# earth-insights/ZoomEarth

Hardware: AMD Instinct MI355X
Metric: questions/sec end-to-end, ZoomEarth-3B on 5000px tiles (higher is better)
Workload: dtype bf16

## Files before the change

### zoomearth_amd/csrc/ze_elementwise.hip

```cpp
#include <hip/hip_fp16.h>

#include "ze_kernels.h"
#include "ze_prng.h"

__device__ __forceinline__ int map_row(int r, int mode, int offset) {
    return mode == 0 ? offset + r : (r >> 4) * 32 + (r & 15) + offset;
}

__global__ void __launch_bounds__(256) k_pack_rows(const void* __restrict__ src, int dtype, int row0, int nrows,
                                                   int cols, bf16_t* __restrict__ dst, int ld, int mode, int offset) {
    const size_t i = (size_t)blockIdx.x * 256 + threadIdx.x;
    if (i >= (size_t)nrows * cols) return;
    const int r = (int)(i / cols), c = (int)(i % cols);
    bf16_t v;
    if (dtype == ZE_BF16) {
        v = ((const bf16_t*)src)[i];
    } else if (dtype == ZE_F16) {
        v = f32_to_bf16(__half2float(((const __half*)src)[i]));
    } else {
        v = f32_to_bf16(((const float*)src)[i]);
    }
    dst[(size_t)map_row(row0 + r, mode, offset) * ld + c] = v;
}

// ... 401 lines not shown
}
void ze_launch_mrope_kv(bf16_t* qkv, int T, int heads, int kv_heads, int D, const bf16_t* cosT, const bf16_t* sinT,
                        const int* pos3, const int* axis_of, bf16_t* kcache, bf16_t* vcache, int max_ctx, int past,
                        const int* row_aux, size_t cache_seq_stride, hipStream_t s, int q_skip) {
    const size_t total = (size_t)T * (heads + 2 * kv_heads) * (D / 2);
    if (total == 0) return;
    if (D % 16 == 0 && mrope_vec_ok) {
        const size_t tv = (size_t)T * (q_skip ? 2 * kv_heads : heads + 2 * kv_heads) * (D / 2) / 8;
        k_mrope_kv_vec<<<(unsigned)((tv + 255) / 256), 256, 0, s>>>(qkv, T, heads, kv_heads, D, cosT, sinT, pos3, axis_of, kcache,
                                                                  vcache, max_ctx, past, row_aux, cache_seq_stride, q_skip);
        return;
    }
    k_mrope_kv<<<(unsigned)((total + 255) / 256), 256, 0, s>>>(qkv, T, heads, kv_heads, D, cosT, sinT, pos3,
                                                               axis_of, kcache, vcache, max_ctx, past, row_aux,
                                                               cache_seq_stride);
}

__global__ void __launch_bounds__(256) k_embed_rows(const int* __restrict__ src, const bf16_t* __restrict__ embed,
                                                    const bf16_t* __restrict__ image_embeds,
                                                    bf16_t* __restrict__ out, int T, int hidden) {
    const int nv = hidden >> 3;
    const size_t i = (size_t)blockIdx.x * 256 + threadIdx.x;
    if (i >= (size_t)T * nv) return;
    const int t = (int)(i / nv), v = (int)(i % nv);
    const int sidx = src[t];
    const bf16_t* row = sidx >= 0 ? embed + (size_t)sidx * hidden : image_embeds + (size_t)(-1 - sidx) * hidden;
    *reinterpret_cast<uint4*>(out + (size_t)t * hidden + v * 8) = *reinterpret_cast<const uint4*>(row + v * 8);
}
void ze_launch_embed_rows(const int* src, const bf16_t* embed, const bf16_t* image_embeds, bf16_t* out, int T,
                          int hidden, hipStream_t s) {
    const size_t n = (size_t)T * (hidden / 8);
    if (n == 0) return;
    k_embed_rows<<<(unsigned)((n + 255) / 256), 256, 0, s>>>(src, embed, image_embeds, out, T, hidden);
}

__global__ void __launch_bounds__(256) k_scatter_rows(const bf16_t* __restrict__ src, int lds_,
                                                      const int* __restrict__ dst_idx, bf16_t* __restrict__ dst,
                                                      int ldd, int rows, int cols) {
    const int nv = cols >> 3;
    const size_t i = (size_t)blockIdx.x * 256 + threadIdx.x;
    if (i >= (size_t)rows * nv) return;
    const int r = (int)(i / nv), v = (int)(i % nv);
    const int d = dst_idx ? dst_idx[r] : r;
    *reinterpret_cast<uint4*>(dst + (size_t)d * ldd + v * 8) =
        *reinterpret_cast<const uint4*>(src + (size_t)r * lds_ + v * 8);
}
void ze_launch_scatter_rows(const bf16_t* src, int lds_, const int* dst_idx, bf16_t* dst, int ldd, int rows,
                            int cols, hipStream_t s) {
    const size_t n = (size_t)rows * (cols / 8);
    if (n == 0) return;
    k_scatter_rows<<<(unsigned)((n + 255) / 256), 256, 0, s>>>(src, lds_, dst_idx, dst, ldd, rows, cols);
}

__global__ void __launch_bounds__(256) k_embed_tokens_batch(const ze_seq_dev* __restrict__ st,
                                                            const int* __restrict__ seq_ids, int n,
                                                            const bf16_t* __restrict__ embed, bf16_t* __restrict__ out,
                                                            int hidden) {
    const int nv = hidden >> 3;
    const size_t i = (size_t)blockIdx.x * 256 + threadIdx.x;
    if (i >= (size_t)n * nv) return;
    const int b = (int)(i / nv), v = (int)(i % nv);
    const int tok = st[seq_ids[b]].token;
    *reinterpret_cast<uint4*>(out + (size_t)b * hidden + v * 8) =
        *reinterpret_cast<const uint4*>(embed + (size_t)tok * hidden + v * 8);
}
struct ze_int_pack {
    int v[128];
};
__global__ void k_set_ints(int* __restrict__ dst, ze_int_pack p, int n) {
    const int i = threadIdx.x;
    if (i < n) dst[i] = p.v[i];
}
void ze_launch_set_ints(int* dst, const int* host_vals, int n, hipStream_t s) {
    for (int o = 0; o < n; o += 128) {
        ze_int_pack p;
        const int m = n - o < 128 ? n - o : 128;
        for (int i = 0; i < 128; ++i) p.v[i] = i < m ? host_vals[o + i] : 0;
        hipLaunchKernelGGL(k_set_ints, dim3(1), dim3(128), 0, s, dst + o, p, m);
    }
}

__global__ void k_scatter_ints(int* __restrict__ dst, ze_int_pack p, int n) {
    const int i = threadIdx.x;
    if (i < n) dst[p.v[i]] = p.v[64 + i];
}
void ze_launch_scatter_ints(int* dst, const int* host_idx, const int* host_vals, int n, hipStream_t s) {
    for (int o = 0; o < n; o += 64) {
        ze_int_pack p;
        const int m = n - o < 64 ? n - o : 64;
        for (int i = 0; i < 64; ++i) {
            p.v[i] = i < m ? host_idx[o + i] : 0;
            p.v[64 + i] = i < m ? host_vals[o + i] : 0;
        }
        hipLaunchKernelGGL(k_scatter_ints, dim3(1), dim3(64), 0, s, dst, p, m);
    }
}

void ze_launch_embed_tokens_batch(const ze_seq_dev* st, const int* seq_ids, int n, const bf16_t* embed, bf16_t* out,
                                  int hidden, hipStream_t s) {
    const size_t tot = (size_t)n * (hidden / 8);
    if (tot == 0) return;
    k_embed_tokens_batch<<<(unsigned)((tot + 255) / 256), 256, 0, s>>>(st, seq_ids, n, embed, out, hidden);
}

__global__ void __launch_bounds__(256) k_rope_kv_batch(bf16_t* __restrict__ qkv, int n, int heads, int kv_heads, int D,
                                                       const bf16_t* __restrict__ cosT, const bf16_t* __restrict__ sinT,
// ... 109 lines not shown
```

### zoomearth_amd/csrc/ze_engine.h

```cpp
#pragma once
#include <algorithm>
#include <map>
#include <tuple>
#include <set>
#include <string>
#include <vector>

#include "ze_host.h"
#include "ze_kernels.h"

struct ze_linear {
    bf16_t* w = nullptr;
    bf16_t* bias = nullptr;
    int n = 0, k = 0, ld = 0;
    uint8_t* w8 = nullptr;
    float* scale8 = nullptr;
    int ld8 = 0;
    bf16_t* wf = nullptr;
    bf16_t* wp = nullptr;
    bf16_t* bias_p = nullptr;
    uint8_t* wf8 = nullptr;
};
struct ze_vit_block {
    bf16_t *norm1 = nullptr, *norm2 = nullptr;
// ... 201 lines not shown
    struct ev_pair { int phase; hipEvent_t a, b; };
    std::vector<ev_pair> ev_used;
    std::vector<ev_pair> ev_free;
    float phase_ms[5] = {0, 0, 0, 0, 0};

    bf16_t* kc(int layer, int seq) const {
        return kcache + (((size_t)layer * cfg.max_seqs + seq) * cfg.kv_heads) * (size_t)cfg.max_ctx * head_dim;
    }
    bf16_t* vc(int layer, int seq) const {
        return vcache + (((size_t)layer * cfg.max_seqs + seq) * cfg.kv_heads) * (size_t)cfg.max_ctx * head_dim;
    }
};

#define ZE_TRY(x)               \
    do {                        \
        int _r = (x);           \
        if (_r != 0) return _r; \
    } while (0)
#define ZE_KCHECK() ZE_HIP(hipGetLastError())

extern unsigned ze_tune_epoch;
void ze_weights_changed(ze_engine* e);
int ze_engine_build_layout(ze_engine* e);
int ze_timer_begin(ze_engine* e, int phase, hipStream_t s);
void ze_timer_end(ze_engine* e, int handle, hipStream_t s);

template <typename T>
static int dev_alloc(ze_engine* e, T** p, size_t count, bool zero = true) {
    ZE_HIP(hipMalloc((void**)p, std::max<size_t>(count, 1) * sizeof(T)));
    if (zero) ZE_HIP(hipMemset(*p, 0, std::max<size_t>(count, 1) * sizeof(T)));
    return 0;
}
static inline int check_seq(ze_engine* e, int seq) {
    if (!e) return ze_fail(e, ZE_ERR_INVALID, "null engine");
    if (seq < 0 || seq >= e->cfg.max_seqs) return ze_fail(e, ZE_ERR_NOTFOUND, "sequence id out of range");
    return ZE_OK;
}

#pragma GCC visibility push(hidden)
int ze_requests_create(ze_engine* e);
void ze_requests_free(ze_engine* e);
void ze_requests_clear(ze_engine* e, int seq, hipStream_t s);
const float* ze_requests_rows(ze_engine* e, const float* logits, const int* seq_ids, int slot0, int n, hipStream_t s);
void ze_requests_logprobs(ze_engine* e, const float* logits, const int* seq_ids, int slot0, int n, hipStream_t s);
void ze_requests_after_token(ze_engine* e, const float* logits, const int* seq_ids, int slot0, int n, hipStream_t s);
int ze_check_filter(ze_engine* e, int top_k, float top_p, float min_p);
void ze_attach_filters(ze_engine* e, ze_sample_opts& so, bool batch);
float ze_penalty_of(const ze_engine* e, const ze_gen_params* p, int seq);
ze_sample_opts ze_sample_opts_of(ze_engine* e, const ze_gen_params* p, int slot, bool batch = false);
ze_step_key ze_step_key_of(const ze_engine* e, int n, int seq, float penalty, int ignore_eos, const ze_sample_opts& so);

enum { ZE_PROJ_QKV = 0, ZE_PROJ_O = 1, ZE_PROJ_GATE_UP = 2, ZE_PROJ_DOWN = 3 };
enum { ZE_NORM_IN = 0, ZE_NORM_POST = 1, ZE_NORM_FINAL = 2 };
void prefill_projection(ze_engine* e, const ze_text_layer& L, int which, int rows, bool norm, bf16_t* out, int ldo, hipStream_t s);
ze_gemv_args gemv_args_of(const ze_engine* e, const ze_linear& lin, int N, int K, const bf16_t* x);
ze_linear lm_head_linear(const ze_engine* e, bool decode);
void batch_norm(ze_engine* e, int li, int n, int which, hipStream_t s);
bool batch_qkv(ze_engine* e, int li, int n, hipStream_t s);
void batch_attention(ze_engine* e, int li, int n, hipStream_t s);
bool batch_o(ze_engine* e, int li, int n, hipStream_t s);
bool batch_gate_up(ze_engine* e, int li, int n, hipStream_t s);
bool batch_down(ze_engine* e, int li, int n, hipStream_t s);
bool batch_lm_head(ze_engine* e, int li, int n, hipStream_t s);
int ensure_fragments(ze_engine* e, hipStream_t s);
void sync_prefix(ze_engine* e, const int32_t* seqs, int n, hipStream_t s);
void upload_mates(ze_engine* e, const int32_t* seqs, int n, hipStream_t s);
void set_live_parts(ze_engine* e, const int32_t* seqs, int n, int steps);
#pragma GCC visibility pop
```

### zoomearth_amd/csrc/ze_engine.hip

```cpp
#include <math.h>
#include <string.h>

#include "ze_engine.h"
#include "ze_prng.h"

thread_local std::string ze_global_error;
extern int ze_mrope_vec_ok;
unsigned ze_tune_epoch = 0;
extern int ze_live_engines;
static int ze_bound_device = -1;

void ze_weights_changed(ze_engine* e) {
    e->frag_ready = false;
    if (e->fp8_ready) {
        e->fp8_ready = false;
        e->fp8_act = false;
        for (auto& L : e->tl)
            for (ze_linear* l : {&L.qkv, &L.o, &L.gate_up, &L.down}) {
                l->w8 = nullptr;
                l->scale8 = nullptr;
                l->wf8 = nullptr;
            }
        e->lm_head8.w8 = nullptr;
        e->lm_head8.scale8 = nullptr;
// ... 245 lines not shown
    e->graphs.assign(c.max_seqs, nullptr);
    e->graph_key.assign(c.max_seqs, ze_step_key{});
    chk(ze_requests_create(e));

    const size_t side = (size_t)std::max(c.max_tile_side, 1024);
    e->fe_tmp_bytes = side * 4096 * 3;
    e->fe_img_bytes = (size_t)4096 * 4096 * 3;
    chk(dev_alloc(e, &e->fe_tmp, e->fe_tmp_bytes, false));
    chk(dev_alloc(e, &e->fe_img, e->fe_img_bytes, false));
    e->fe_coef_ints = (size_t)4096 * 96 * 2 + 4096 * 4;
    chk(dev_alloc(e, &e->fe_coef, e->fe_coef_ints, false));
    if (r == 0 && hipHostMalloc((void**)&e->fe_coef_host, e->fe_coef_ints * sizeof(int)) != hipSuccess)
        r = ze_fail(e, ZE_ERR_HIP, "hipHostMalloc failed");

    const size_t np = c.max_patches;
    const int vh = c.vit_hidden, mu = c.spatial_merge_size * c.spatial_merge_size;
    const int pk = c.in_channels * c.temporal_patch_size * c.patch_size * c.patch_size;
    chk(dev_alloc(e, &e->vx, np * pk));
    chk(dev_alloc(e, &e->vh, np * vh));
    chk(dev_alloc(e, &e->vy, np * vh));
    chk(dev_alloc(e, &e->vqkv, np * 3 * vh));
    chk(dev_alloc(e, &e->vo, np * vh));
    chk(dev_alloc(e, &e->va, np * e->vit_ipad));
    chk(dev_alloc(e, &e->vz, np / mu * (size_t)vh * mu + 8));
    chk(dev_alloc(e, &e->vz2, np / mu * (size_t)c.vit_out_hidden + 8));
    chk(dev_alloc(e, &e->vcos, np * (e->vit_head_dim / 2)));
    chk(dev_alloc(e, &e->vsin, np * (e->vit_head_dim / 2)));
    chk(dev_alloc(e, &e->vperm, np));
    chk(dev_alloc(e, &e->vinv, np));
    chk(dev_alloc(e, &e->vtiles_win, np));
    chk(dev_alloc(e, &e->vtiles_full, np));
    e->v_host_ints_cap = np * 2 + np * 4 * 2 + 64;
    e->v_host_f32_cap = np * e->vit_head_dim;
    if (r == 0 && (hipHostMalloc((void**)&e->v_host_ints, e->v_host_ints_cap * sizeof(int)) != hipSuccess ||
                   hipHostMalloc((void**)&e->v_host_f32, e->v_host_f32_cap * sizeof(float)) != hipSuccess))
        r = ze_fail(e, ZE_ERR_HIP, "hipHostMalloc failed");

    const size_t tm = std::max(c.max_ctx, c.max_prefill_rows);
    e->prefill_rows = (int)tm;
    const int nqkv = (c.heads + 2 * c.kv_heads) * e->head_dim;
    chk(dev_alloc(e, &e->th, tm * c.hidden));
    chk(dev_alloc(e, &e->ty, tm * c.hidden));
    chk(dev_alloc(e, &e->ty8p, tm * c.hidden, false));
    chk(dev_alloc(e, &e->ty8p_scale, tm, false));
    chk(dev_alloc(e, &e->damax, 2 * 2048));
    if (r == 0 && e->damax) ze_launch_amax_init(e->damax, nullptr);
    chk(dev_alloc(e, &e->ty8, (size_t)64 * c.hidden));
    chk(dev_alloc(e, &e->ty8_scale, 64));
    chk(dev_alloc(e, &e->tqkv, tm * nqkv));
    chk(dev_alloc(e, &e->to, tm * c.heads * e->head_dim));
    chk(dev_alloc(e, &e->ta, tm * e->text_ipad));
    chk(dev_alloc(e, &e->tsrc, tm));
    chk(dev_alloc(e, &e->tpos, tm * 3));
    const size_t ntile_cap = tm / 64 + c.max_seqs + 2;
    chk(dev_alloc(e, &e->ttiles, ntile_cap));
    chk(dev_alloc(e, &e->ttile_aux, ntile_cap * 2));
    chk(dev_alloc(e, &e->trow_aux, tm * 2));
    e->t_host_ints_cap = tm * 6 + ntile_cap * 6 + 64;
    if (r == 0 && hipHostMalloc((void**)&e->t_host_ints, e->t_host_ints_cap * sizeof(int)) != hipSuccess)
        r = ze_fail(e, ZE_ERR_HIP, "hipHostMalloc failed");

    chk(dev_alloc(e, &e->dh, c.hidden));
    chk(dev_alloc(e, &e->dq, (size_t)c.heads * e->head_dim));
    chk(dev_alloc(e, &e->dattn, (size_t)c.heads * e->head_dim));
    chk(dev_alloc(e, &e->dact, e->text_ipad));
    chk(dev_alloc(e, &e->dlogits, (size_t)c.max_seqs * c.vocab));
    {
        const size_t rows_pad = ((size_t)std::max(c.max_seqs, 64) + 255) / 256 * 256;
        const size_t slab_floats = std::max((size_t)24 << 20, (size_t)400 * 64 * rows_pad);
        const int ticket_cap = std::max(4096, (int)(200 * (rows_pad / 64)) + 64);
        chk(dev_alloc(e, &e->gslab, slab_floats, false));
        chk(dev_alloc(e, &e->gtickets, (size_t)ticket_cap, true));
        e->gslab_floats = slab_floats;
        e->gticket_cap = ticket_cap;
    }
    {
        const size_t br = (size_t)(std::max(c.max_seqs, 64) + 63) / 64 * 64;
        chk(dev_alloc(e, &e->bh, br * c.hidden));
        chk(dev_alloc(e, &e->by, br * c.hidden));
        chk(dev_alloc(e, &e->bqkv, br * nqkv));
        chk(dev_alloc(e, &e->bo, br * c.heads * e->head_dim));
        chk(dev_alloc(e, &e->ba, br * e->text_ipad));
    }
    chk(dev_alloc(e, &e->bseq, c.max_seqs));
    chk(dev_alloc(e, &e->bmate, c.max_seqs));
    chk(dev_alloc(e, &e->blogits, (size_t)c.max_seqs * c.vocab));
    chk(dev_alloc(e, &e->bpartial, (size_t)c.max_seqs * std::max(e->max_splits, 8) * c.heads * 132));
    chk(dev_alloc(e, &e->bsample, (size_t)c.max_seqs * 3 * 128 + 8));
    if (r == 0 && hipHostMalloc((void**)&e->bstate_host, sizeof(ze_seq_dev) * c.max_seqs) != hipSuccess)
        r = ze_fail(e, ZE_ERR_HIP, "hipHostMalloc failed");
    chk(dev_alloc(e, &e->dpartial, (size_t)e->max_splits * c.heads * 132));
    chk(dev_alloc(e, &e->dsample, 2 * 128 + 64 + 128 + 8));
    chk(dev_alloc(e, &e->atickets, (size_t)c.max_seqs * c.kv_heads));
    if (r == 0 && hipHostMalloc((void**)&e->d_host_ints, (64 + c.max_seqs) * sizeof(int)) != hipSuccess)
        r = ze_fail(e, ZE_ERR_HIP, "hipHostMalloc failed");
    e->staging_bytes = (size_t)64 << 20;
    if (r == 0 && hipMalloc(&e->staging, e->staging_bytes) != hipSuccess) r = ze_fail(e, ZE_ERR_HIP, "hipMalloc staging");

    if (r != 0) {
        ze_global_error = e->err;
        ze_engine_destroy(e);
        return r;
    }
    e->counted = true;
    __atomic_add_fetch(&ze_live_engines, 1, __ATOMIC_RELAXED);
    *out = e;
    return ZE_OK;
// ... 212 lines not shown
```

### zoomearth_amd/csrc/ze_forward.hip

```cpp
#include <math.h>
#include <cmath>
#include <string.h>

#include <algorithm>

#include "ze_engine.h"

extern int ze_gemv_knobs[24];

static int frontend_acquire(ze_engine* e) {
    if (e->fe_in_flight) {
        ZE_HIP(hipEventSynchronize(e->fe_done));
        e->fe_in_flight = false;
    }
    return ZE_OK;
}
static int frontend_release(ze_engine* e, hipStream_t s) {
    if (!e->fe_done) ZE_HIP(hipEventCreateWithFlags(&e->fe_done, hipEventDisableTiming));
    ZE_HIP(hipEventRecord(e->fe_done, s));
    e->fe_in_flight = true;
    return ZE_OK;
}
static int stage_acquire(ze_engine* e, hipEvent_t& ev) {
    if (ev) ZE_HIP(hipEventSynchronize(ev));
// ... 456 lines not shown
    if (hipMalloc((void**)&d, want * sizeof(int)) != hipSuccess) {
        hipHostFree(h);
        return ze_fail(e, ZE_ERR_NOMEM, "hipMalloc of the id transfer scratch failed");
    }
    host = h;
    dev = d;
    cap = want;
    return ZE_OK;
}

extern "C" int ze_seq_mark_seen_batch(ze_engine* e, const int32_t* seqs, const int32_t* counts, int n, const int32_t* ids, void* stream) {
    if (!e || n < 0 || (n > 0 && (!seqs || !counts))) return ze_fail(e, ZE_ERR_INVALID, "bad arguments");
    if (n == 0) return ZE_OK;
    if (n > e->cfg.max_seqs) return ze_fail(e, ZE_ERR_INVALID, "more chains than slots");
    size_t total = 0;
    int max_count = 0;
    for (int i = 0; i < n; ++i) {
        ZE_TRY(check_seq(e, seqs[i]));
        if (counts[i] < 0 || counts[i] > e->cfg.max_ctx) return ze_fail(e, ZE_ERR_INVALID, "bad id count");
        total += (size_t)counts[i];
        max_count = std::max(max_count, counts[i]);
    }
    if (total > 0 && !ids) return ze_fail(e, ZE_ERR_INVALID, "bad ids");
    for (size_t i = 0; i < total; ++i)
        if (ids[i] < 0 || ids[i] >= e->cfg.vocab) return ze_fail(e, ZE_ERR_INVALID, "token id out of range");
    if (total == 0) return ZE_OK;
    hipSetDevice(e->device);
    hipStream_t s = (hipStream_t)stream;
    ZE_TRY(stage_acquire(e, e->xs_staged));
    ZE_TRY(xfer_reserve(e, e->xs_host, e->xs_dev, e->xs_cap, (size_t)(2 * n + 1) + total, e->xs_staged, s));
    int* h = e->xs_host;
    h[0] = 0;
    for (int i = 0; i < n; ++i) {
        h[i + 1] = h[i] + counts[i];
        h[n + 1 + i] = seqs[i];
    }
    memcpy(h + 2 * n + 1, ids, total * sizeof(int));
    ZE_HIP(hipMemcpyAsync(e->xs_dev, h, ((size_t)(2 * n + 1) + total) * sizeof(int), hipMemcpyHostToDevice, s));
    ze_launch_mark_seen_batch(e->seen, e->cfg.vocab, e->xs_dev, e->xs_dev + 2 * n + 1, n, max_count, s);
    ZE_KCHECK();
    ZE_TRY(stage_release(e, e->xs_staged, s));
    return ZE_OK;
}

static void note_split(ze_engine* e, int seq, const int32_t* ids, int len, int past) {
    if (e->split_host[seq] != 0 || e->cfg.vision_end_token_id < 0) return;
    for (int t = 0; t < len; ++t)
        if (ids[t] == e->cfg.vision_end_token_id) {
            if (past + t + 1 < 65536) e->split_host[seq] = past + t + 1;
            return;
        }
}

static void prefill_norm_gemm(ze_engine* e, const bf16_t* norm_w, const ze_linear& lin, const bf16_t* bias, int epi, bf16_t* out,
                              int ldo, int rows, int N, hipStream_t s) {
    const ze_config& c = e->cfg;
    const int H = c.hidden;
    if (e->fp8_act && lin.w8 && ze_gemv_knobs[12] != 1 && H % 128 == 0 && H >= 256 && lin.ld8 % 16 == 0) {
        if (norm_w) ze_launch_rmsnorm(e->th, H, norm_w, e->ty, H, rows, H, c.rms_eps, s, 0, 3, e->ty8p, e->ty8p_scale);
        if (ze_launch_gemm_mx(epi, e->ty8p, H, e->ty8p_scale, lin.w8, lin.ld8, lin.scale8, bias, out, ldo, rows, N, H, s)) return;
    }
    if (norm_w) ze_launch_rmsnorm(e->th, H, norm_w, e->ty, H, rows, H, c.rms_eps, s, 0, e->fp8_act ? 1 : 0);
    ze_launch_gemm(epi, e->ty, H, lin.w, lin.ld, bias, nullptr, 0, out, ldo, nullptr, rows, N, H, s, e->prefill_ws());
}

void prefill_projection(ze_engine* e, const ze_text_layer& L, int which, int rows, bool norm, bf16_t* out, int ldo, hipStream_t s) {
    const int H = e->cfg.hidden, nq = e->cfg.heads * e->head_dim, nqkv = nq + 2 * e->cfg.kv_heads * e->head_dim, ip = e->text_ipad;
    switch (which) {
        case ZE_PROJ_QKV:
            prefill_norm_gemm(e, norm ? L.in_norm : nullptr, L.qkv, L.qkv.bias, ZE_EPI_NONE, out, ldo, rows, nqkv, s);
            break;
        case ZE_PROJ_O:
            ze_launch_gemm(ZE_EPI_RESIDUAL, e->to, nq, L.o.w, L.o.ld, nullptr, e->th, H, out, ldo, nullptr, rows, H, nq, s, e->prefill_ws());
            break;
        case ZE_PROJ_GATE_UP:
            prefill_norm_gemm(e, norm ? L.post_norm : nullptr, L.gate_up, nullptr, ZE_EPI_SWIGLU, out, ldo, rows, 2 * ip, s);
            break;
        default:
            ze_launch_gemm(ZE_EPI_RESIDUAL, e->ta, ip, L.down.w, L.down.ld, nullptr, e->th, H, out, ldo, nullptr, rows, H, ip, s, e->prefill_ws());
            break;
    }
}

static int prefill_bq() { return (ze_gemv_knobs[1] == 9 || ze_gemv_knobs[1] == 7) ? 64 : ZE_FA_BQ_LONG; }

struct prefill_kv {
    int slot;
    int past;
    const int* row_aux;
    const int* tile_aux;
    size_t seq_stride;
    int n_tiles;
    int rope_rows;
};

static void prefill_layers(ze_engine* e, int rows, const prefill_kv& kv, hipStream_t s) {
    const ze_config& c = e->cfg;
    const int H = c.hidden, hd = e->head_dim, nq = c.heads * hd, nqkv = nq + 2 * c.kv_heads * hd;
    const float scale = 1.0f / sqrtf((float)hd);
    const int bq = prefill_bq();
    const bool q_in_flash = hd == 128 && ze_mrope_vec_ok != 0 && ze_gemv_knobs[22] != 1;
    const ze_fa_rope rope = q_in_flash ? ze_fa_rope{e->cosT, e->sinT, e->tpos, c.mrope_section[0], c.mrope_section[0] + c.mrope_section[1], kv.rope_rows}
                                       : ze_fa_rope{nullptr, nullptr, nullptr, 0, 0, 0};
    for (int li = 0; li < c.layers; ++li) {
        const ze_text_layer& L = e->tl[li];
        bf16_t *k = e->kc(li, kv.slot), *v = e->vc(li, kv.slot);
        prefill_projection(e, L, ZE_PROJ_QKV, rows, true, e->tqkv, nqkv, s);
        ze_launch_mrope_kv(e->tqkv, rows, c.heads, c.kv_heads, hd, e->cosT, e->sinT, e->tpos, e->axis_of, k, v, c.max_ctx, kv.past,
                           kv.row_aux, kv.seq_stride, s, q_in_flash ? 1 : 0);
        ze_launch_flash_attn(hd, 1, e->tqkv, nqkv, hd, k, hd, c.max_ctx * hd, v, hd, c.max_ctx * hd, e->to, nq, hd, e->ttiles, kv.n_tiles,
                             c.heads, c.heads / c.kv_heads, scale, kv.past, s, kv.tile_aux, kv.seq_stride, bq, 0, rope);
        prefill_projection(e, L, ZE_PROJ_O, rows, true, e->th, H, s);
        prefill_projection(e, L, ZE_PROJ_GATE_UP, rows, true, e->ta, e->text_ipad, s);
        prefill_projection(e, L, ZE_PROJ_DOWN, rows, true, e->th, H, s);
    }
}

ze_linear lm_head_linear(const ze_engine* e, bool decode) {
    ze_linear l;
    l.w = e->lm_head;
    l.ld = e->cfg.hidden;
    if (decode) {
        l.w8 = e->lm_head8.w8;
        l.scale8 = e->lm_head8.scale8;
        l.ld8 = e->lm_head8.ld8;
    }
    return l;
}

ze_gemv_args gemv_args_of(const ze_engine* e, const ze_linear& lin, int N, int K, const bf16_t* x) {
    ze_gemv_args a;
    memset(&a, 0, sizeof(a));
    a.W = lin.w;
    a.ldw = lin.ld;
    if (e->fp8_ready && lin.w8) {
        a.W8 = lin.w8;
        a.scale8 = lin.scale8;
        a.ldw8 = lin.ld8;
    }
    a.N = N;
    a.K = K;
    a.x = x;
    a.D = e->head_dim;
    return a;
}

static void prefill_logits(ze_engine* e, const bf16_t* const* x, float* const* out, int n, hipStream_t s) {
    const ze_config& c = e->cfg;
    if (ze_launch_logits_rows(e->lm_head, c.hidden, c.vocab, c.hidden, e->final_norm, c.rms_eps, x, out, n, s)) return;
    for (int i = 0; i < n; ++i) {
        ze_gemv_args a = gemv_args_of(e, lm_head_linear(e, false), c.vocab, c.hidden, x[i]);
        a.norm_w = e->final_norm;
        a.eps = c.rms_eps;
        a.out_f32 = out[i];
        ze_launch_gemv(ZE_GV_LOGITS, a, s);
    }
}

static int stage_chain(ze_engine* e, const int32_t* ids, const int32_t* position_ids, int len, int row0, int total, int* src, int* pos,
                       int& img) {
    const ze_config& c = e->cfg;
    for (int t = row0; t < row0 + len; ++t) {
        const int id = ids[t];
        if (id < 0 || id >= c.vocab) return ze_fail(e, ZE_ERR_INVALID, "token id out of range");
        src[t] = (id == c.image_token_id) ? -1 - img++ : id;
        for (int a = 0; a < 3; ++a) {
            const int p = position_ids[(size_t)a * total + t];
            if (p < 0 || p >= e->max_pos) return ze_fail(e, ZE_ERR_INVALID, "position id out of range");
            pos[(size_t)a * total + t] = p;
        }
    }
    return ZE_OK;
}

static int stage_tiles(int* tiles, int nt, int row0, int len, int past) {
    const int bq = prefill_bq();
    for (int q0 = 0; q0 < len; q0 += bq, ++nt) {
        tiles[4 * nt + 0] = row0 + q0;
        tiles[4 * nt + 1] = row0 + std::min(q0 + bq, len);
        tiles[4 * nt + 2] = 0;
        tiles[4 * nt + 3] = past + len;
    }
    return nt;
}

static int image_mismatch(ze_engine* e, int tokens, int features) {
    return ze_fail(e, ZE_ERR_MISMATCH, "Image features and image tokens do not match, tokens: " + std::to_string(tokens) +
                                           ", features: " + std::to_string(features));
}

static int prefill_impl(ze_engine* e, int seq, const int32_t* input_ids, int len, const void* image_embeds,
                        int n_image_rows, const int32_t* position_ids, int rope_delta, float* out_logits,
                        float* out_logps, void* stream) {
    ZE_TRY(check_seq(e, seq));
    if (!input_ids || !position_ids || len <= 0) return ze_fail(e, ZE_ERR_INVALID, "bad prefill arguments");
    const ze_config& c = e->cfg;
    const int past = e->ctx_host[seq];
    if (past + len > c.max_ctx) return ze_fail(e, ZE_ERR_NOMEM, "sequence exceeds max_ctx");
    hipStream_t s = (hipStream_t)stream;
    hipSetDevice(e->device);
    const int H = c.hidden;

    ZE_TRY(stage_acquire(e, e->t_staged));
    int* src = e->t_host_ints;
    int* pos = src + len;
    int* tiles = pos + 3 * len;
    int img = 0;
    ZE_TRY(stage_chain(e, input_ids, position_ids, len, 0, len, src, pos, img));
    if (img != n_image_rows || (img > 0 && !image_embeds)) return image_mismatch(e, img, n_image_rows);
    note_split(e, seq, input_ids, len, past);
    const int nt = stage_tiles(tiles, 0, 0, len, past);
    ZE_HIP(hipMemcpyAsync(e->tsrc, src, (size_t)len * sizeof(int), hipMemcpyHostToDevice, s));
    ZE_HIP(hipMemcpyAsync(e->tpos, pos, (size_t)3 * len * sizeof(int), hipMemcpyHostToDevice, s));
    ZE_HIP(hipMemcpyAsync(e->ttiles, tiles, (size_t)nt * 16, hipMemcpyHostToDevice, s));
    ZE_TRY(stage_release(e, e->t_staged, s));

    const int th = ze_timer_begin(e, 2, s);
    ze_launch_embed_rows(e->tsrc, e->embed, (const bf16_t*)image_embeds, e->th, len, H, s);
    prefill_layers(e, len, prefill_kv{seq, past, nullptr, nullptr, 0, nt, len}, s);
    {
        const bf16_t* xr = e->th + (size_t)(len - 1) * H;
        float* lo = e->dlogits + (size_t)seq * c.vocab;
        prefill_logits(e, &xr, &lo, 1, s);
    }
    if (out_logps && len > 1) {
        const int ldl = (c.vocab + 7) & ~7;
        int chunk = (int)std::min<size_t>((size_t)e->prefill_rows * e->text_ipad / ldl, (size_t)len - 1);
        if (chunk >= 128) chunk &= ~127;
        if (chunk < 1) return ze_fail(e, ZE_ERR_NOMEM, "prefill workspace too small for one row of logits");
        ZE_HIP(hipMemcpyAsync(e->trow_aux, input_ids + 1, (size_t)(len - 1) * sizeof(int), hipMemcpyHostToDevice, s));
        ze_launch_rmsnorm(e->th, H, e->final_norm, e->ty, H, len - 1, H, c.rms_eps, s);
        for (int r0 = 0; r0 < len - 1; r0 += chunk) {
            const int m = std::min(chunk, len - 1 - r0);
            ze_launch_gemm(ZE_EPI_NONE, e->ty + (size_t)r0 * H, H, e->lm_head, H, nullptr, nullptr, 0, e->ta, ldl,
                           nullptr, m, c.vocab, H, s);
            ze_launch_token_logprob(e->ta, ldl, c.vocab, e->trow_aux + r0, out_logps + r0, m, s);
        }
    }
    ze_timer_end(e, th, s);
    ZE_KCHECK();
    if (out_logits)
        ZE_HIP(hipMemcpyAsync(out_logits, e->dlogits + (size_t)seq * c.vocab, (size_t)c.vocab * sizeof(float),
                              hipMemcpyDeviceToDevice, s));
    e->ctx_host[seq] = past + len;
    e->delta_host[seq] = rope_delta;
    return push_state(e, seq, s, input_ids[len - 1], 0, 0);
}

extern "C" int ze_prefill(ze_engine* e, int seq, const int32_t* input_ids, int len, const void* image_embeds,
                          int n_image_rows, const int32_t* position_ids, int rope_delta, float* out_logits,
                          void* stream) {
    return prefill_impl(e, seq, input_ids, len, image_embeds, n_image_rows, position_ids, rope_delta, out_logits,
                        nullptr, stream);
}

extern "C" int ze_score(ze_engine* e, int seq, const int32_t* input_ids, int len, const void* image_embeds,
                        int n_image_rows, const int32_t* position_ids, int rope_delta, float* out_logps,
                        void* stream) {
    if (!out_logps) return ze_fail(e, ZE_ERR_INVALID, "ze_score needs an output buffer");
    return prefill_impl(e, seq, input_ids, len, image_embeds, n_image_rows, position_ids, rope_delta, nullptr,
                        out_logps, stream);
}

extern "C" int ze_prefill_batch(ze_engine* e, const int32_t* seqs, int n, const int32_t* lens, const int32_t* input_ids,
                                const void* image_embeds, const int32_t* n_image_rows, const int32_t* position_ids,
                                const int32_t* rope_deltas, void* stream) {
    if (!e || !seqs || !lens || !input_ids || !position_ids || !rope_deltas || n <= 0)
        return ze_fail(e, ZE_ERR_INVALID, "bad prefill arguments");
    const ze_config& c = e->cfg;
    hipStream_t s = (hipStream_t)stream;
    hipSetDevice(e->device);
    const int H = c.hidden;
    int total = 0;
    for (int i = 0; i < n; ++i) {
        ZE_TRY(check_seq(e, seqs[i]));
        for (int k2 = 0; k2 < i; ++k2)
            if (seqs[k2] == seqs[i]) return ze_fail(e, ZE_ERR_INVALID, "a chain appears twice in the batch");
        if (lens[i] <= 0) return ze_fail(e, ZE_ERR_INVALID, "bad prefill arguments");
        if (e->ctx_host[seqs[i]] + lens[i] > c.max_ctx) return ze_fail(e, ZE_ERR_NOMEM, "sequence exceeds max_ctx");
        total += lens[i];
    }
    if (total > e->prefill_rows) return ze_fail(e, ZE_ERR_NOMEM, "batched prefill exceeds max_prefill_rows");

    ZE_TRY(stage_acquire(e, e->t_staged));
    int* src = e->t_host_ints;
    int* pos = src + total;
    int* row_aux = pos + 3 * total;
    int* tiles = row_aux + 2 * total;
    int img = 0, nt = 0, row0 = 0;
    std::vector<int> tile_aux;
    for (int i = 0; i < n; ++i) {
        const int seq = seqs[i], len = lens[i], past = e->ctx_host[seq], img0 = img;
        ZE_TRY(stage_chain(e, input_ids, position_ids, len, row0, total, src, pos, img));
        for (int t = 0; t < len; ++t) {
            row_aux[2 * (row0 + t)] = seq;
            row_aux[2 * (row0 + t) + 1] = past + t;
        }
        note_split(e, seq, input_ids + row0, len, past);
        const int want = n_image_rows ? n_image_rows[i] : 0;
        if (img - img0 != want || (img > img0 && !image_embeds)) return image_mismatch(e, img - img0, want);
        const int nt0 = nt;
        nt = stage_tiles(tiles, nt, row0, len, past);
        for (int t = nt0; t < nt; ++t) {
            tile_aux.push_back(seq);
            tile_aux.push_back(past - row0);
        }
        row0 += len;
    }
    int* taux = tiles + 4 * nt;
    memcpy(taux, tile_aux.data(), tile_aux.size() * sizeof(int));
    ZE_HIP(hipMemcpyAsync(e->tsrc, src, (size_t)total * sizeof(int), hipMemcpyHostToDevice, s));
    ZE_HIP(hipMemcpyAsync(e->tpos, pos, (size_t)3 * total * sizeof(int), hipMemcpyHostToDevice, s));
    ZE_HIP(hipMemcpyAsync(e->trow_aux, row_aux, (size_t)2 * total * sizeof(int), hipMemcpyHostToDevice, s));
    ZE_HIP(hipMemcpyAsync(e->ttiles, tiles, (size_t)nt * 16, hipMemcpyHostToDevice, s));
    ZE_HIP(hipMemcpyAsync(e->ttile_aux, taux, (size_t)nt * 2 * sizeof(int), hipMemcpyHostToDevice, s));
    ZE_TRY(stage_release(e, e->t_staged, s));

    const int th = ze_timer_begin(e, 2, s);
    ze_launch_embed_rows(e->tsrc, e->embed, (const bf16_t*)image_embeds, e->th, total, H, s);
    prefill_layers(e, total, prefill_kv{0, 0, e->trow_aux, e->ttile_aux, (size_t)c.kv_heads * c.max_ctx * e->head_dim, nt, total}, s);
    {
        std::vector<const bf16_t*> xr(n);
        std::vector<float*> lo(n);
        row0 = 0;
        for (int i = 0; i < n; ++i) {
            xr[i] = e->th + (size_t)(row0 + lens[i] - 1) * H;
            lo[i] = e->dlogits + (size_t)seqs[i] * c.vocab;
            row0 += lens[i];
        }
        prefill_logits(e, xr.data(), lo.data(), n, s);
    }
    ze_timer_end(e, th, s);
    ZE_KCHECK();
    row0 = 0;
    for (int i = 0; i < n; ++i) {
        e->ctx_host[seqs[i]] += lens[i];
        e->delta_host[seqs[i]] = rope_deltas[i];
        ZE_TRY(push_state(e, seqs[i], s, input_ids[row0 + lens[i] - 1], 0, 0));
        row0 += lens[i];
    }
    return ZE_OK;
}

static int ze_enqueue_decode_step(ze_engine* e, int seq, float penalty, int ignore_eos, bool sample, const ze_sample_opts& so,
                                  hipStream_t s) {
    const ze_config& c = e->cfg;
    const int H = c.hidden, hd = e->head_dim, nq = c.heads * hd, nqkv = nq + 2 * c.kv_heads * hd;
    const ze_seq_dev* st = e->st_dev + seq;
    const float scale = 1.0f / sqrtf((float)hd);
    for (int li = 0; li < c.layers; ++li) {
        const ze_text_layer& L = e->tl[li];
        ze_gemv_args a = gemv_args_of(e, L.qkv, nqkv, H, e->dh);
        a.norm_w = L.in_norm;
        a.eps = c.rms_eps;
        a.bias = L.qkv.bias;
        a.out_bf16 = e->dq;
        a.st = st;
        a.cosT = e->cosT;
        a.sinT = e->sinT;
        a.kcache = e->kc(li, seq);
        a.vcache = e->vc(li, seq);
        a.heads = c.heads;
        a.kv_heads = c.kv_heads;
        a.max_ctx = c.max_ctx;
        a.act8 = e->fp8_act ? 1 : 0;
        if (li == 0) {
            a.embed = e->embed;
            a.embed_out = e->dh;
        }
        ze_launch_gemv(ZE_GV_QKV_ROPE, a, s);
        ze_launch_attn_decode(e->dq, 0, e->kc(li, seq), e->vc(li, seq), 0, e->dattn, 0, st, nullptr, 1, c.heads,
                              c.kv_heads, hd, c.max_ctx, scale, e->dpartial, e->max_splits, e->atickets, s);
        ze_gemv_args o = gemv_args_of(e, L.o, H, nq, e->dattn);
        o.out_bf16 = e->dh;
        ze_launch_gemv(ZE_GV_RESIDUAL, o, s);
        ze_gemv_args g = gemv_args_of(e, L.gate_up, 2 * e->text_ipad, H, e->dh);
        g.norm_w = L.post_norm;
        g.eps = c.rms_eps;
        g.out_bf16 = e->dact;
// ... 1384 lines not shown
```

### zoomearth_amd/csrc/ze_kernels.h

```cpp
#pragma once
#include "ze_common.h"

enum { ZE_EPI_NONE = 0, ZE_EPI_GELU = 1, ZE_EPI_RESIDUAL = 2, ZE_EPI_SWIGLU = 3, ZE_EPI_F32 = 4, ZE_EPI_QKV_ROPE = 5 };
enum { ZE_GV_QKV_ROPE = 0, ZE_GV_RESIDUAL = 1, ZE_GV_SWIGLU = 2, ZE_GV_LOGITS = 3, ZE_GV_PLAIN = 4 };

#if defined(__HIPCC__)
__device__ __forceinline__ int ze_kv_swz(int row) {
#ifdef ZE_KV_SWZ_OLD
    return ((row & 3) << 2) | ((row >> 2) & 3);
#else
    const int hi = (row >> 3) & 1;
    return ((((row & 7) ^ (hi << 2)) << 1) | hi);
#endif
}
#endif

#if defined(__HIPCC__)
__device__ __forceinline__ void rope8(const uint4& a, const uint4& b, const uint4& c4, const uint4& s4, uint4& o1, uint4& o2) {
    const uint32_t* pa = reinterpret_cast<const uint32_t*>(&a);
    const uint32_t* pb = reinterpret_cast<const uint32_t*>(&b);
    const uint32_t* pc = reinterpret_cast<const uint32_t*>(&c4);
    const uint32_t* ps = reinterpret_cast<const uint32_t*>(&s4);
    uint32_t r1[4], r2[4];
#pragma unroll
// ... 30 lines not shown
    int32_t stream;
    int32_t split;
};

void ze_launch_resize_h(const uint8_t* src, int src_h, int src_w, int bx0, int by0, int box_h, uint8_t* dst,
                        int out_w, const int* xmin, const int* xcnt, const int* kk, int ksize, int max_span,
                        hipStream_t s, int inside = 0);
void ze_launch_resize_v(const uint8_t* src, int src_h, int src_w, int bx0, int by0, int row_bytes, uint8_t* dst,
                        int out_h, const int* ymin, const int* ycnt, const int* kk, int ksize, int boxed,
                        hipStream_t s);
void ze_launch_crop(const uint8_t* src, int src_h, int src_w, int bx0, int by0, uint8_t* dst, int out_h, int out_w,
                    hipStream_t s);
void ze_launch_patchify(const uint8_t* img, int h, int w, const float* lut, float* out, int P, int M, int T, int C,
                        hipStream_t s);

void ze_launch_pack_rows(const void* src, int dtype, int row0, int nrows, int cols, bf16_t* dst, int ld, int mode,
                         int offset, hipStream_t s);
void ze_launch_fill_rows(uint64_t seed, float c_scale, float base, int rows, int cols, bf16_t* dst, int ld, int mode,
                         int offset, hipStream_t s);
struct ze_gemm_ws {
    float* slab = nullptr;
    size_t slab_floats = 0;
    unsigned* tickets = nullptr;
    int ticket_cap = 0;
};
void ze_launch_rmsnorm(const bf16_t* x, int ldx, const bf16_t* w, bf16_t* y, int ldy, int rows, int cols, float eps,
                       hipStream_t s, int frag = 0, int act8 = 0, uint8_t* y8 = nullptr, float* yscale = nullptr);
void ze_launch_pack_fragments(const bf16_t* W, int ldw, int n, int k, bf16_t* Wf, hipStream_t s, int rope_dim = 0);
void ze_launch_gemm_oneshot(int epi, const bf16_t* Xf, const bf16_t* Wf, const bf16_t* bias, const bf16_t* R, int ldr,
                            bf16_t* C, int ldc, int M, int N, int K, hipStream_t s, const float* wscale = nullptr,
                            const float* ascale = nullptr);
void ze_launch_qkv_rope_oneshot(const bf16_t* Xf, const bf16_t* Wf_perm, const bf16_t* bias, bf16_t* q_out, int ldq, int M,
                                int K, int heads, int kv_heads, const bf16_t* cosT, const bf16_t* sinT,
                                const ze_seq_dev* st, const int* seq_ids, bf16_t* kcache, bf16_t* vcache,
                                size_t cache_seq_stride, int max_ctx, hipStream_t s, const float* wscale = nullptr,
                                const float* ascale = nullptr);
bool ze_launch_gemm_mx(int epi, const uint8_t* A, int lda, const float* sa, const uint8_t* W, int ldw, const float* sw,
                       const bf16_t* bias, bf16_t* C, int ldc, int M, int N, int K, hipStream_t s);
void ze_launch_gemm_frag(int epi, const bf16_t* Xf, const bf16_t* Wf, const bf16_t* bias, const bf16_t* R, int ldr,
                         bf16_t* C, int ldc, int M, int N, int K, hipStream_t s, const float* wscale = nullptr,
                         const float* ascale = nullptr);
void ze_launch_pack_fragments8(const uint8_t* W8, int ld8, int n, int k, uint8_t* Wf8, hipStream_t s, int rope_dim = 0);
void ze_launch_gather_cast_rows(const float* src, int k, const int* perm, bf16_t* dst, int kp, int rows,
                                hipStream_t s);
void ze_launch_vision_rope(bf16_t* qkv, const float* cosT, const float* sinT, int n, int heads, int D, hipStream_t s);
void ze_launch_mrope_kv(bf16_t* qkv, int T, int heads, int kv_heads, int D, const bf16_t* cosT, const bf16_t* sinT,
                        const int* pos3, const int* axis_of, bf16_t* kcache, bf16_t* vcache, int max_ctx, int past, const int* row_aux, size_t cache_seq_stride,
                        hipStream_t s, int q_skip = 0);
extern int ze_mrope_vec_ok;
void ze_launch_embed_rows(const int* src, const bf16_t* embed, const bf16_t* image_embeds, bf16_t* out, int T,
                          int hidden, hipStream_t s);
void ze_launch_scatter_rows(const bf16_t* src, int lds_, const int* dst_idx, bf16_t* dst, int ldd, int rows, int cols,
                            hipStream_t s);

struct ze_qkv_epi {
    const ze_seq_dev* st;
    const int* seq_ids;
    const bf16_t* cosT;
    const bf16_t* sinT;
    bf16_t* kcache;
    bf16_t* vcache;
    size_t cache_seq_stride;
    int max_ctx, heads, kv_heads, pad_;
};
void ze_launch_permute_qkv(const bf16_t* W, int ldw, const bf16_t* bias, int n_heads_total, int K, bf16_t* Wp, bf16_t* bias_p, hipStream_t s);
void ze_launch_gemm_qkv_rope(const bf16_t* A, int lda, const bf16_t* Wp, int ldw, const bf16_t* bias_p, const ze_qkv_epi* dev_args,
                             bf16_t* C, int ldc, int M, int N, int K, hipStream_t s);

void ze_launch_gemm(int epi, const bf16_t* A, int lda, const bf16_t* W, int ldw, const bf16_t* bias, const bf16_t* R,
                    int ldr, bf16_t* C, int ldc, const int* c_rows, int M, int N, int K, hipStream_t s, const ze_gemm_ws& ws = ze_gemm_ws());

void ze_launch_gemm_stream(int epi, const bf16_t* A, int lda, const bf16_t* W, int ldw, const bf16_t* bias,
                           const bf16_t* R, int ldr, bf16_t* C, int ldc, int M, int N, int K, const ze_gemm_ws& ws,
                           hipStream_t s);
void ze_launch_gemm_wide(int epi, const bf16_t* A, int lda, const bf16_t* W, int ldw, const bf16_t* bias, const bf16_t* R,
                         int ldr, bf16_t* C, int ldc, int M, int N, int K, const ze_gemm_ws& ws, hipStream_t s);

void ze_launch_gemm_p8(int epi, const bf16_t* A, int lda, const bf16_t* W, int ldw, const bf16_t* bias, const bf16_t* R, int ldr,
                       bf16_t* C, int ldc, const int* c_rows, int M, int N, int K, hipStream_t s, const ze_gemm_ws& ws = ze_gemm_ws());

struct ze_gemv_args {
    const bf16_t* W;
    int ldw, N, K;
    const bf16_t* x;
    const bf16_t* norm_w;
    float eps;
    const bf16_t* bias;
    bf16_t* out_bf16;
    float* out_f32;
    const ze_seq_dev* st;
    const bf16_t* cosT;
    const bf16_t* sinT;
    bf16_t* kcache;
    bf16_t* vcache;
    int heads, kv_heads, D, max_ctx;
    const bf16_t* embed;
    bf16_t* embed_out;
    const uint8_t* W8;
    const float* scale8;
    int ldw8;
    int act8;
    const uint8_t* seen;
    float penalty;
    float* amax_ws;
};
bool ze_launch_gemv(int epi, const ze_gemv_args& a, hipStream_t s);
// ... 150 lines not shown
```

Before: 70.13.

## Compute only last-token rows in final prefill layer after KV write

In the last text layer of prefill, K/V are still written for every row, but attention, the O projection and the MLP run only for the rows whose logits are needed: the final token of each sequence. Per-row attention tiles and gather indices are staged on the host. Kept hidden and output rows are gathered into a scratch region carved from the MLP buffer. This avoids a full layer of O/gate_up/down GEMMs and attention over every prompt row. In exchange it adds tile staging, a larger tile buffer allocation and aliasing of scratch space within the activation buffer. The path is disabled when log-probs over all rows are requested.

Result: no change. 70.11 (-0.0%).

```diff
diff --git a/zoomearth_amd/csrc/ze_elementwise.hip b/zoomearth_amd/csrc/ze_elementwise.hip
--- a/zoomearth_amd/csrc/ze_elementwise.hip
+++ b/zoomearth_amd/csrc/ze_elementwise.hip
@@ -477,6 +477,23 @@
     k_scatter_rows<<<(unsigned)((n + 255) / 256), 256, 0, s>>>(src, lds_, dst_idx, dst, ldd, rows, cols);
 }
 
+__global__ void __launch_bounds__(256) k_gather_rows(const bf16_t* __restrict__ src, int lds_,
+                                                     const int* __restrict__ src_idx, bf16_t* __restrict__ dst,
+                                                     int ldd, int rows, int cols) {
+    const int nv = cols >> 3;
+    const size_t i = (size_t)blockIdx.x * 256 + threadIdx.x;
+    if (i >= (size_t)rows * nv) return;
+    const int r = (int)(i / nv), v = (int)(i % nv);
+    *reinterpret_cast<uint4*>(dst + (size_t)r * ldd + v * 8) =
+        *reinterpret_cast<const uint4*>(src + (size_t)src_idx[r] * lds_ + v * 8);
+}
+void ze_launch_gather_rows(const bf16_t* src, int lds_, const int* src_idx, bf16_t* dst, int ldd, int rows, int cols,
+                           hipStream_t s) {
+    const size_t n = (size_t)rows * (cols / 8);
+    if (n == 0) return;
+    k_gather_rows<<<(unsigned)((n + 255) / 256), 256, 0, s>>>(src, lds_, src_idx, dst, ldd, rows, cols);
+}
+
 __global__ void __launch_bounds__(256) k_embed_tokens_batch(const ze_seq_dev* __restrict__ st,
                                                             const int* __restrict__ seq_ids, int n,
                                                             const bf16_t* __restrict__ embed, bf16_t* __restrict__ out,
diff --git a/zoomearth_amd/csrc/ze_engine.h b/zoomearth_amd/csrc/ze_engine.h
--- a/zoomearth_amd/csrc/ze_engine.h
+++ b/zoomearth_amd/csrc/ze_engine.h
@@ -277,7 +277,11 @@
 
 enum { ZE_PROJ_QKV = 0, ZE_PROJ_O = 1, ZE_PROJ_GATE_UP = 2, ZE_PROJ_DOWN = 3 };
 enum { ZE_NORM_IN = 0, ZE_NORM_POST = 1, ZE_NORM_FINAL = 2 };
-void prefill_projection(ze_engine* e, const ze_text_layer& L, int which, int rows, bool norm, bf16_t* out, int ldo, hipStream_t s);
+struct ze_prefill_rows {
+    bf16_t *h, *o, *a;
+};
+void prefill_projection(ze_engine* e, const ze_text_layer& L, int which, int rows, bool norm, bf16_t* out, int ldo, hipStream_t s,
+                        const ze_prefill_rows* at = nullptr);
 ze_gemv_args gemv_args_of(const ze_engine* e, const ze_linear& lin, int N, int K, const bf16_t* x);
 ze_linear lm_head_linear(const ze_engine* e, bool decode);
 void batch_norm(ze_engine* e, int li, int n, int which, hipStream_t s);
diff --git a/zoomearth_amd/csrc/ze_engine.hip b/zoomearth_amd/csrc/ze_engine.hip
--- a/zoomearth_amd/csrc/ze_engine.hip
+++ b/zoomearth_amd/csrc/ze_engine.hip
@@ -321,7 +321,7 @@
     chk(dev_alloc(e, &e->ta, tm * e->text_ipad));
     chk(dev_alloc(e, &e->tsrc, tm));
     chk(dev_alloc(e, &e->tpos, tm * 3));
-    const size_t ntile_cap = tm / 64 + c.max_seqs + 2;
+    const size_t ntile_cap = tm / 64 + 3 * (size_t)c.max_seqs + 4;
     chk(dev_alloc(e, &e->ttiles, ntile_cap));
     chk(dev_alloc(e, &e->ttile_aux, ntile_cap * 2));
     chk(dev_alloc(e, &e->trow_aux, tm * 2));
diff --git a/zoomearth_amd/csrc/ze_forward.hip b/zoomearth_amd/csrc/ze_forward.hip
--- a/zoomearth_amd/csrc/ze_forward.hip
+++ b/zoomearth_amd/csrc/ze_forward.hip
@@ -532,32 +532,35 @@
         }
 }
 
-static void prefill_norm_gemm(ze_engine* e, const bf16_t* norm_w, const ze_linear& lin, const bf16_t* bias, int epi, bf16_t* out,
-                              int ldo, int rows, int N, hipStream_t s) {
+static void prefill_norm_gemm(ze_engine* e, const bf16_t* x, const bf16_t* norm_w, const ze_linear& lin, const bf16_t* bias, int epi,
+                              bf16_t* out, int ldo, int rows, int N, hipStream_t s) {
     const ze_config& c = e->cfg;
     const int H = c.hidden;
     if (e->fp8_act && lin.w8 && ze_gemv_knobs[12] != 1 && H % 128 == 0 && H >= 256 && lin.ld8 % 16 == 0) {
-        if (norm_w) ze_launch_rmsnorm(e->th, H, norm_w, e->ty, H, rows, H, c.rms_eps, s, 0, 3, e->ty8p, e->ty8p_scale);
+        if (norm_w) ze_launch_rmsnorm(x, H, norm_w, e->ty, H, rows, H, c.rms_eps, s, 0, 3, e->ty8p, e->ty8p_scale);
         if (ze_launch_gemm_mx(epi, e->ty8p, H, e->ty8p_scale, lin.w8, lin.ld8, lin.scale8, bias, out, ldo, rows, N, H, s)) return;
     }
-    if (norm_w) ze_launch_rmsnorm(e->th, H, norm_w, e->ty, H, rows, H, c.rms_eps, s, 0, e->fp8_act ? 1 : 0);
+    if (norm_w) ze_launch_rmsnorm(x, H, norm_w, e->ty, H, rows, H, c.rms_eps, s, 0, e->fp8_act ? 1 : 0);
     ze_launch_gemm(epi, e->ty, H, lin.w, lin.ld, bias, nullptr, 0, out, ldo, nullptr, rows, N, H, s, e->prefill_ws());
 }
 
-void prefill_projection(ze_engine* e, const ze_text_layer& L, int which, int rows, bool norm, bf16_t* out, int ldo, hipStream_t s) {
+void prefill_projection(ze_engine* e, const ze_text_layer& L, int which, int rows, bool norm, bf16_t* out, int ldo, hipStream_t s,
+                        const ze_prefill_rows* at) {
     const int H = e->cfg.hidden, nq = e->cfg.heads * e->head_dim, nqkv = nq + 2 * e->cfg.kv_heads * e->head_dim, ip = e->text_ipad;
+    const ze_prefill_rows own{e->th, e->to, e->ta};
+    const ze_prefill_rows& r = at ? *at : own;
     switch (which) {
         case ZE_PROJ_QKV:
-            prefill_norm_gemm(e, norm ? L.in_norm : nullptr, L.qkv, L.qkv.bias, ZE_EPI_NONE, out, ldo, rows, nqkv, s);
+            prefill_norm_gemm(e, r.h, norm ? L.in_norm : nullptr, L.qkv, L.qkv.bias, ZE_EPI_NONE, out, ldo, rows, nqkv, s);
             break;
         case ZE_PROJ_O:
-            ze_launch_gemm(ZE_EPI_RESIDUAL, e->to, nq, L.o.w, L.o.ld, nullptr, e->th, H, out, ldo, nullptr, rows, H, nq, s, e->prefill_ws());
+            ze_launch_gemm(ZE_EPI_RESIDUAL, r.o, nq, L.o.w, L.o.ld, nullptr, r.h, H, out, ldo, nullptr, rows, H, nq, s, e->prefill_ws());
             break;
         case ZE_PROJ_GATE_UP:
-            prefill_norm_gemm(e, norm ? L.post_norm : nullptr, L.gate_up, nullptr, ZE_EPI_SWIGLU, out, ldo, rows, 2 * ip, s);
+            prefill_norm_gemm(e, r.h, norm ? L.post_norm : nullptr, L.gate_up, nullptr, ZE_EPI_SWIGLU, out, ldo, rows, 2 * ip, s);
             break;
         default:
-            ze_launch_gemm(ZE_EPI_RESIDUAL, e->ta, ip, L.down.w, L.down.ld, nullptr, e->th, H, out, ldo, nullptr, rows, H, ip, s, e->prefill_ws());
+            ze_launch_gemm(ZE_EPI_RESIDUAL, r.a, ip, L.down.w, L.down.ld, nullptr, r.h, H, out, ldo, nullptr, rows, H, ip, s, e->prefill_ws());
             break;
     }
 }
@@ -572,9 +575,22 @@
     size_t seq_stride;
     int n_tiles;
     int rope_rows;
+    int n_keep = 0;
+    const int* keep_rows = nullptr;
+    const int4* keep_tiles = nullptr;
+    const int* keep_tile_aux = nullptr;
 };
 
-static void prefill_layers(ze_engine* e, int rows, const prefill_kv& kv, hipStream_t s) {
+static ze_prefill_rows prefill_kept_rows(const ze_engine* e, int n) {
+    const size_t a = ((size_t)n * e->text_ipad + 63) & ~(size_t)63, h = ((size_t)n * e->cfg.hidden + 63) & ~(size_t)63;
+    return ze_prefill_rows{e->ta + a, e->ta + a + h, e->ta};
+}
+static bool prefill_kept_rows_fit(const ze_engine* e, int n) {
+    const size_t need = (size_t)n * ((size_t)e->text_ipad + e->cfg.hidden + (size_t)e->cfg.heads * e->head_dim) + 128;
+    return need <= (size_t)e->prefill_rows * e->text_ipad && e->cfg.hidden % 8 == 0 && e->text_ipad % 8 == 0 && e->head_dim % 8 == 0;
+}
+
+static const bf16_t* prefill_layers(ze_engine* e, int rows, const prefill_kv& kv, hipStream_t s) {
     const ze_config& c = e->cfg;
     const int H = c.hidden, hd = e->head_dim, nq = c.heads * hd, nqkv = nq + 2 * c.kv_heads * hd;
     const float scale = 1.0f / sqrtf((float)hd);
@@ -582,18 +598,31 @@
     const bool q_in_flash = hd == 128 && ze_mrope_vec_ok != 0 && ze_gemv_knobs[22] != 1;
     const ze_fa_rope rope = q_in_flash ? ze_fa_rope{e->cosT, e->sinT, e->tpos, c.mrope_section[0], c.mrope_section[0] + c.mrope_section[1], kv.rope_rows}
                                        : ze_fa_rope{nullptr, nullptr, nullptr, 0, 0, 0};
+    const bool kept = kv.n_keep > 0 && kv.n_keep < rows && ze_gemv_knobs[22] != 2 && prefill_kept_rows_fit(e, kv.n_keep);
     for (int li = 0; li < c.layers; ++li) {
         const ze_text_layer& L = e->tl[li];
         bf16_t *k = e->kc(li, kv.slot), *v = e->vc(li, kv.slot);
         prefill_projection(e, L, ZE_PROJ_QKV, rows, true, e->tqkv, nqkv, s);
         ze_launch_mrope_kv(e->tqkv, rows, c.heads, c.kv_heads, hd, e->cosT, e->sinT, e->tpos, e->axis_of, k, v, c.max_ctx, kv.past,
                            kv.row_aux, kv.seq_stride, s, q_in_flash ? 1 : 0);
+        if (kept && li == c.layers - 1) {
+            const ze_prefill_rows r = prefill_kept_rows(e, kv.n_keep);
+            ze_launch_flash_attn(hd, 1, e->tqkv, nqkv, hd, k, hd, c.max_ctx * hd, v, hd, c.max_ctx * hd, e->to, nq, hd, kv.keep_tiles,
+                                 kv.n_keep, c.heads, c.heads / c.kv_heads, scale, kv.past, s, kv.keep_tile_aux, kv.seq_stride, 64, 0, rope);
+            ze_launch_gather_rows(e->to, nq, kv.keep_rows, r.o, nq, kv.n_keep, nq, s);
+            ze_launch_gather_rows(e->th, H, kv.keep_rows, r.h, H, kv.n_keep, H, s);
+            prefill_projection(e, L, ZE_PROJ_O, kv.n_keep, true, r.h, H, s, &r);
+            prefill_projection(e, L, ZE_PROJ_GATE_UP, kv.n_keep, true, r.a, e->text_ipad, s, &r);
+            prefill_projection(e, L, ZE_PROJ_DOWN, kv.n_keep, true, r.h, H, s, &r);
+            return r.h;
+        }
         ze_launch_flash_attn(hd, 1, e->tqkv, nqkv, hd, k, hd, c.max_ctx * hd, v, hd, c.max_ctx * hd, e->to, nq, hd, e->ttiles, kv.n_tiles,
                              c.heads, c.heads / c.kv_heads, scale, kv.past, s, kv.tile_aux, kv.seq_stride, bq, 0, rope);
         prefill_projection(e, L, ZE_PROJ_O, rows, true, e->th, H, s);
         prefill_projection(e, L, ZE_PROJ_GATE_UP, rows, true, e->ta, e->text_ipad, s);
         prefill_projection(e, L, ZE_PROJ_DOWN, rows, true, e->th, H, s);
     }
+    return e->th;
 }
 
 ze_linear lm_head_linear(const ze_engine* e, bool decode) {
@@ -664,6 +693,18 @@
     return nt;
 }
 
+static int stage_kept_rows(int* tiles, int nt, const int* rows, const int* kv1, int n) {
+    for (int i = 0; i < n; ++i) {
+        tiles[4 * (nt + i) + 0] = rows[i];
+        tiles[4 * (nt + i) + 1] = rows[i] + 1;
+        tiles[4 * (nt + i) + 2] = 0;
+        tiles[4 * (nt + i) + 3] = kv1[i];
+    }
+    const int slots = (n + 3) / 4;
+    for (int i = 0; i < 4 * slots; ++i) tiles[4 * (nt + n) + i] = i < n ? rows[i] : 0;
+    return nt + n + slots;
+}
+
 static int image_mismatch(ze_engine* e, int tokens, int features) {
     return ze_fail(e, ZE_ERR_MISMATCH, "Image features and image tokens do not match, tokens: " + std::to_string(tokens) +
                                            ", features: " + std::to_string(features));
@@ -690,16 +731,19 @@
     if (img != n_image_rows || (img > 0 && !image_embeds)) return image_mismatch(e, img, n_image_rows);
     note_split(e, seq, input_ids, len, past);
     const int nt = stage_tiles(tiles, 0, 0, len, past);
+    const int n_keep = out_logps ? 0 : 1, last_row = len - 1, last_kv1 = past + len;
+    const int slots = n_keep ? stage_kept_rows(tiles, nt, &last_row, &last_kv1, 1) : nt;
     ZE_HIP(hipMemcpyAsync(e->tsrc, src, (size_t)len * sizeof(int), hipMemcpyHostToDevice, s));
     ZE_HIP(hipMemcpyAsync(e->tpos, pos, (size_t)3 * len * sizeof(int), hipMemcpyHostToDevice, s));
-    ZE_HIP(hipMemcpyAsync(e->ttiles, tiles, (size_t)nt * 16, hipMemcpyHostToDevice, s));
+    ZE_HIP(hipMemcpyAsync(e->ttiles, tiles, (size_t)slots * 16, hipMemcpyHostToDevice, s));
     ZE_TRY(stage_release(e, e->t_staged, s));
 
     const int th = ze_timer_begin(e, 2, s);
     ze_launch_embed_rows(e->tsrc, e->embed, (const bf16_t*)image_embeds, e->th, len, H, s);
-    prefill_layers(e, len, prefill_kv{seq, past, nullptr, nullptr, 0, nt, len}, s);
+    const bf16_t* hl = prefill_layers(e, len, prefill_kv{seq, past, nullptr, nullptr, 0, nt, len, n_keep, (const int*)(e->ttiles + nt + n_keep),
+                                                         e->ttiles + nt, nullptr}, s);
     {
-        const bf16_t* xr = e->th + (size_t)(len - 1) * H;
+        const bf16_t* xr = hl == e->th ? e->th + (size_t)(len - 1) * H : hl;
         float* lo = e->dlogits + (size_t)seq * c.vocab;
         prefill_logits(e, &xr, &lo, 1, s);
     }
@@ -768,9 +812,13 @@
     int* row_aux = pos + 3 * total;
     int* tiles = row_aux + 2 * total;
     int img = 0, nt = 0, row0 = 0;
-    std::vector<int> tile_aux;
+    std::vector<int> tile_aux, keep_row(n), keep_kv1(n), keep_aux;
     for (int i = 0; i < n; ++i) {
         const int seq = seqs[i], len = lens[i], past = e->ctx_host[seq], img0 = img;
+        keep_row[i] = row0 + len - 1;
+        keep_kv1[i] = past + len;
+        keep_aux.push_back(seq);
+        keep_aux.push_back(past - row0);
         ZE_TRY(stage_chain(e, input_ids, position_ids, len, row0, total, src, pos, img));
         for (int t = 0; t < len; ++t) {
             row_aux[2 * (row0 + t)] = seq;
@@ -787,24 +835,27 @@
         }
         row0 += len;
     }
-    int* taux = tiles + 4 * nt;
+    const int slots = stage_kept_rows(tiles, nt, keep_row.data(), keep_kv1.data(), n);
+    int* taux = tiles + 4 * slots;
     memcpy(taux, tile_aux.data(), tile_aux.size() * sizeof(int));
+    memcpy(taux + 2 * nt, keep_aux.data(), keep_aux.size() * sizeof(int));
     ZE_HIP(hipMemcpyAsync(e->tsrc, src, (size_t)total * sizeof(int), hipMemcpyHostToDevice, s));
     ZE_HIP(hipMemcpyAsync(e->tpos, pos, (size_t)3 * total * sizeof(int), hipMemcpyHostToDevice, s));
     ZE_HIP(hipMemcpyAsync(e->trow_aux, row_aux, (size_t)2 * total * sizeof(int), hipMemcpyHostToDevice, s));
-    ZE_HIP(hipMemcpyAsync(e->ttiles, tiles, (size_t)nt * 16, hipMemcpyHostToDevice, s));
-    ZE_HIP(hipMemcpyAsync(e->ttile_aux, taux, (size_t)nt * 2 * sizeof(int), hipMemcpyHostToDevice, s));
+    ZE_HIP(hipMemcpyAsync(e->ttiles, tiles, (size_t)slots * 16, hipMemcpyHostToDevice, s));
+    ZE_HIP(hipMemcpyAsync(e->ttile_aux, taux, (size_t)(nt + n) * 2 * sizeof(int), hipMemcpyHostToDevice, s));
     ZE_TRY(stage_release(e, e->t_staged, s));
 
     const int th = ze_timer_begin(e, 2, s);
     ze_launch_embed_rows(e->tsrc, e->embed, (const bf16_t*)image_embeds, e->th, total, H, s);
-    prefill_layers(e, total, prefill_kv{0, 0, e->trow_aux, e->ttile_aux, (size_t)c.kv_heads * c.max_ctx * e->head_dim, nt, total}, s);
+    const bf16_t* hl = prefill_layers(e, total, prefill_kv{0, 0, e->trow_aux, e->ttile_aux, (size_t)c.kv_heads * c.max_ctx * e->head_dim, nt, total,
+                                                           n, (const int*)(e->ttiles + nt + n), e->ttiles + nt, e->ttile_aux + 2 * nt}, s);
     {
         std::vector<const bf16_t*> xr(n);
         std::vector<float*> lo(n);
         row0 = 0;
         for (int i = 0; i < n; ++i) {
-            xr[i] = e->th + (size_t)(row0 + lens[i] - 1) * H;
+            xr[i] = hl == e->th ? e->th + (size_t)(row0 + lens[i] - 1) * H : hl + (size_t)i * H;
             lo[i] = e->dlogits + (size_t)seqs[i] * c.vocab;
             row0 += lens[i];
         }
diff --git a/zoomearth_amd/csrc/ze_kernels.h b/zoomearth_amd/csrc/ze_kernels.h
--- a/zoomearth_amd/csrc/ze_kernels.h
+++ b/zoomearth_amd/csrc/ze_kernels.h
@@ -106,6 +106,8 @@
                           int hidden, hipStream_t s);
 void ze_launch_scatter_rows(const bf16_t* src, int lds_, const int* dst_idx, bf16_t* dst, int ldd, int rows, int cols,
                             hipStream_t s);
+void ze_launch_gather_rows(const bf16_t* src, int lds_, const int* src_idx, bf16_t* dst, int ldd, int rows, int cols,
+                           hipStream_t s);
 
 struct ze_qkv_epi {
     const ze_seq_dev* st;
```
